# Probabilistic-Surgical-Vision/uncertainty-model

Hardware: AMD Instinct MI355X
Metric: stereo-pairs/sec (train step) at 256x512, 1/2/4/8 MI355X; loss delta vs ref (higher is better)
Workload: dtype bf16; 1 GPU; depth+uncertainty train step (BASELINE config 2): fwd+4-scale loss+bwd+Adam; global_batch=8, per_gpu_batch=8, height=256, width=512, loss=bayesian, parallelism=dp1, launch=hip-graph, graph=config.yml (nodes=5 stage graphs)

## Files before the change

### uncertainty-model_amd/csrc/knobs.h

```cpp
#pragma once

#define UM_KNOBS(X)                                                                         \
                                \
                \
  X(small, 1)                                                                               \
                \
                 \
                \
                  \
                           \
  X(small_tiles, 1024)                                                                      \
  X(split_below, 600)                                                                       \
  X(split_target, 1024)                                                                     \
  X(split_minsteps, 4)                                                                      \
                       \
                \
                     \
                  \
                   \
  X(glds_split_below, 256)                                                                  \
  X(glds_split_target, 512)                                                                 \
              \
  X(halo, 1)                                                                                \
  X(halo_min_tiles, 256)                                                                    \
                  \
                     \
  X(halo_max_nc, 192)                                                                       \
                       \
  X(odd_bn, 1)                                                                              \
              \
  X(bk64, 3)                                                                                \
                  \
                   \
                \
                    \
  X(glds, 5)                                                                                \
               \
                      \
                 \
                   \
  X(glds_deep, 3)                                                                           \
  X(glds_deep_blocks, 256)                                                                  \
                 \
                          \
  X(xcd_col, 0)                                                                             \
                 \
               \
             \
  X(tappack, 1)                                                                             \
                     \
  X(cls4, 1)                                                                                \
                  \
                 \
                    \
                \
              \
  X(cls_glds, 3)                                                                            \
                                            \
                   \
                 \
  X(pad_dgrad, 1)                                                                           \
                  \
                 \
                     \
                   \
                                                      \
  X(fold_split_nc, 64)                                                                      \
                                                   \
                             \
  X(halo_pf2, 0)                                                                            \
                    \
                 \
                    \
  X(halo_persist, 1)                                                                        \
  X(halo_grid, 0)                                                                           \
                  \
                   \
  X(halo_res_kb, 48)                                                                        \
                    \
  X(halo_staged, 1)                                                                         \
                    \
                      \
                                                         \
  X(border_valu, 1)                                                                         \
                       \
                        \
  X(s1x1, 1)                                                                                \
                   \
  X(s1x1_small, 1)                                                                          \
               \
                  \
  X(cat_fused, 0)                                                                           \
                   \
  X(merge_ns, 1)                                                                            \
              \
                                    \
  X(colred_single, 131072)                                                                  \
  X(colred_per, 16384)                                                                      \
               \
                                                          \
  X(wtr_tbk, 32)                                                                            \
                            \
  X(w1x1, 1)                                                                                \
               \
  X(border_split, 1)                                                                        \
                   \
  X(up2_valu, 1)                                                                            \
                   \
                                         \
  X(wsplit_blocks, 0)                                                                       \
                     \
  X(wred_t, 1)                                                                              \
                            \
  X(bn_bwd_rows_max, 1024)                                                                  \
                     \
  X(bn_slice, 1)                                                                            \
              \
                                          \
  X(dh_fwd, 0)                                                                              \
  X(dh_fwd128, 1)                                                                           \
               \
  X(dh_dgrad, 1)

namespace umamd {

struct Knobs {
#define UM_KNOB_FIELD(name, dflt) int name;
  UM_KNOBS(UM_KNOB_FIELD)
#undef UM_KNOB_FIELD
  Knobs();
};

Knobs& knobs();

}
```

### uncertainty-model_amd/csrc/wgrad_tr.hip

```cpp
#include <algorithm>
#include <cstdlib>

#include <atomic>

#include "common.h"
#include "wgrad_tr.h"
#include "knobs.h"

namespace {

typedef __attribute__((ext_vector_type(4))) __bf16 bf16x4_t;

constexpr int TBN = 128;

struct TrArgs {
  const bf16_t* x;
  const bf16_t* dy;
  float* slabs;
  int N, H, W, C, ldx, K, R, stride, pad, reflect, P, Q, ldy;
  int M, RRC, m_per_split;
  int row_step;
};

__device__ __forceinline__ int bit(int v, int b) { return (v >> b) & 1; }
template <int NCH>
__device__ __forceinline__ int swz(int row) {
  if (NCH == 8) return bit(row, 0) | (bit(row, 1) << 1) | (bit(row, 3) << 2);
  if (NCH == 4) return bit(row, 1) | (bit(row, 3) << 1);
  return 0;
}
template <int NCH>
__device__ __forceinline__ int img_off(int row, int c8) {
  return row * NCH * 16 + (((c8 >> 1) ^ swz<NCH>(row)) << 4) + ((c8 & 1) << 3);
}

__device__ __forceinline__ bf16x4_t tr_read(const bf16_t* p) {
  return __builtin_amdgcn_ds_read_tr16_b64_v4bf16(
      (__attribute__((address_space(3))) bf16x4_t*)(p));
}

struct Pix {
  int n, p, q;
  bool ok;
};
__device__ __forceinline__ Pix pix_at(long m, int P, int Q, long mend) {
  Pix x;
  x.ok = m < mend;
  const long mm = x.ok ? m : 0;
  const long pq = (long)P * Q;
  x.n = (int)(mm / pq);
  const int r = (int)(mm - x.n * pq);
  x.p = r / Q;
  x.q = r - x.p * Q;
  return x;
}
template <int BM, int TBK>
__global__ void __launch_bounds__(256) wgrad_tr_kernel(TrArgs a) {
  constexpr int NCA = BM / 16, NCB = TBN / 16;
  constexpr int TM = BM / 32, TN = 4;
  constexpr int A_PER = TBK * BM / 8 / 256;
  constexpr int B_PER = TBK * TBN / 8 / 256;
  constexpr int KS = TBK / 32;
  static_assert(A_PER >= 1 && B_PER >= 2 && TBK % 32 == 0, "tiles");
  __shared__ __attribute__((aligned(16))) bf16_t sA[2][TBK * BM];
  __shared__ __attribute__((aligned(16))) bf16_t sB[2][TBK * TBN];

  const int tid = threadIdx.x, lane = tid & 63, wave = tid >> 6;
  const int wm = wave >> 1, wn = wave & 1;
  const int g = lane >> 4, q4 = (lane >> 2) & 3, p4 = lane & 3;
  const int bk = blockIdx.x * BM;
  const int bj = blockIdx.y * TBN;
  const long m_begin = (long)blockIdx.z * a.m_per_split;
  const long m_end = min((long)a.M, m_begin + a.m_per_split);

  const int mlen = (int)(m_end - m_begin);
  int mrel = 0;
  const bf16_t* adp[A_PER];
  int aso[A_PER], alim[A_PER];
  const long astep = (long)TBK * a.ldy;
#pragma unroll
  for (int u = 0; u < A_PER; ++u) {
    const int id = tid + u * 256;
    const int row = id / (BM / 8), c8 = id % (BM / 8);
    aso[u] = img_off<NCA>(row, c8);
    alim[u] = bk + c8 * 8 < a.K ? mlen - row : 0;
    adp[u] = a.dy + (m_begin + row) * a.ldy + bk + c8 * 8;
  }
  const bf16_t* bimg[B_PER];
  int bso[B_PER], blim[B_PER], bp[B_PER], bq[B_PER], by0[B_PER], bx0[B_PER], byo[B_PER],
      bxo[B_PER];
  const long img_stride = (long)a.H * a.W * a.ldx;
  const int row_pitch = a.W * a.ldx;
  auto yoff = [&](int p, int y0) {
    int yy = p * a.stride + y0;
    if (a.reflect) yy = reflect_idx(yy, a.H);
    return (yy < 0 || yy >= a.H) ? -1 : yy * row_pitch;
  };
  auto xoff = [&](int q, int x0) {
    int xx = q * a.stride + x0;
    if (a.reflect) xx = reflect_idx(xx, a.W);
    return (xx < 0 || xx >= a.W) ? -1 : xx * a.ldx;
  };
#pragma unroll
  for (int u = 0; u < B_PER; ++u) {
    const int id = tid + u * 256;
    const int row = id / (TBN / 8), c8 = id % (TBN / 8);
    bso[u] = img_off<NCB>(row, c8);
    const int j = bj + c8 * 8;
    const bool ok = j < a.RRC;
    blim[u] = ok ? mlen - row : 0;
    const int jj = ok ? j : 0;
    const int tap = jj / a.C;
    const int ry = tap / a.R;
    by0[u] = ry - a.pad;
    bx0[u] = tap - ry * a.R - a.pad;
    const Pix px = pix_at(m_begin + row, a.P, a.Q, m_end);
    bp[u] = px.p;
    bq[u] = px.q;
    bimg[u] = a.x + px.n * img_stride + (jj - tap * a.C);
    byo[u] = yoff(bp[u], by0[u]);
    bxo[u] = xoff(bq[u], bx0[u]);
  }

  uint4 ra[A_PER], rb[B_PER];
  auto load = [&]() {
#pragma unroll
    for (int u = 0; u < A_PER; ++u) {
      ra[u] = make_uint4(0, 0, 0, 0);
      if (mrel < alim[u]) ra[u] = *reinterpret_cast<const uint4*>(adp[u]);
    }
#pragma unroll
    for (int u = 0; u < B_PER; ++u) {
      rb[u] = make_uint4(0, 0, 0, 0);
      if (mrel < blim[u] && (byo[u] | bxo[u]) >= 0)
        rb[u] = *reinterpret_cast<const uint4*>(bimg[u] + (byo[u] + bxo[u]));
    }
  };
  auto store = [&](int buf) {
#pragma unroll
    for (int u = 0; u < A_PER; ++u) *reinterpret_cast<uint4*>(&sA[buf][aso[u]]) = ra[u];
#pragma unroll
    for (int u = 0; u < B_PER; ++u) *reinterpret_cast<uint4*>(&sB[buf][bso[u]]) = rb[u];
  };
  auto advance = [&]() {
    mrel += TBK;
#pragma unroll
    for (int u = 0; u < A_PER; ++u) adp[u] += astep;
    const bool rows = a.row_step > 0;
#pragma unroll
    for (int u = 0; u < B_PER; ++u) {
      int p = bp[u], q = bq[u];
      const bf16_t* img = bimg[u];
      if (rows) {
        p += a.row_step;
        if (p >= a.P) {
          p -= a.P;
          img += img_stride;
        }
      } else {
        q += TBK;
        while (q >= a.Q) {
          q -= a.Q;
          if (++p == a.P) {
            p = 0;
            img += img_stride;
          }
        }
      }
      bp[u] = p;
      bq[u] = q;
      bimg[u] = img;
      byo[u] = yoff(p, by0[u]);
      if (!rows) bxo[u] = xoff(q, bx0[u]);
    }
  };

  int oa[TM][2], ob[TN][2];
#pragma unroll
  for (int h = 0; h < 2; ++h) {
    const int row = 8 * g + q4 + 4 * h;
#pragma unroll
    for (int i = 0; i < TM; ++i) {
      const int ct = (wm * (BM / 2) + i * 16) / 16;
      oa[i][h] = row * NCA * 16 + ((ct ^ swz<NCA>(row)) << 4) + 4 * p4;
    }
#pragma unroll
    for (int j = 0; j < TN; ++j) {
      const int ct = (wn * 64 + j * 16) / 16;
      ob[j][h] = row * NCB * 16 + ((ct ^ swz<NCB>(row)) << 4) + 4 * p4;
    }
  }

  f32x4_t acc[TM][TN];
#pragma unroll
  for (int i = 0; i < TM; ++i)
#pragma unroll
    for (int j = 0; j < TN; ++j) acc[i][j] = f32x4_t{0.f, 0.f, 0.f, 0.f};

  if (m_begin < m_end) {
    load();
    store(0);
    advance();
  }
  __syncthreads();
  int cur = 0;
  for (long m0 = m_begin; m0 < m_end; m0 += TBK) {
    const bool more = m0 + TBK < m_end;
    if (more) load();
#pragma unroll
    for (int ks = 0; ks < KS; ++ks) {
      const int da = ks * 32 * NCA * 16, db = ks * 32 * NCB * 16;
      bf16x8_t fa[TM], fb[TN];
#pragma unroll
      for (int i = 0; i < TM; ++i) {
        const bf16x4_t lo = tr_read(&sA[cur][oa[i][0] + da]);
        const bf16x4_t hi = tr_read(&sA[cur][oa[i][1] + da]);
        fa[i] = bf16x8_t{lo[0], lo[1], lo[2], lo[3], hi[0], hi[1], hi[2], hi[3]};
      }
#pragma unroll
      for (int j = 0; j < TN; ++j) {
        const bf16x4_t lo = tr_read(&sB[cur][ob[j][0] + db]);
        const bf16x4_t hi = tr_read(&sB[cur][ob[j][1] + db]);
        fb[j] = bf16x8_t{lo[0], lo[1], lo[2], lo[3], hi[0], hi[1], hi[2], hi[3]};
      }
#pragma unroll
      for (int i = 0; i < TM; ++i)
#pragma unroll
        for (int j = 0; j < TN; ++j)
          acc[i][j] = __builtin_amdgcn_mfma_f32_16x16x32_bf16(fa[i], fb[j], acc[i][j], 0, 0, 0);
    }
    if (more) {
      store(cur ^ 1);
      advance();
    }
    __syncthreads();
    cur ^= 1;
  }

  float* out = a.slabs + (long)blockIdx.z * a.K * a.RRC;
  const int col = lane & 15, row4 = (lane >> 4) * 4;
#pragma unroll
  for (int i = 0; i < TM; ++i)
#pragma unroll
    for (int j = 0; j < TN; ++j)
#pragma unroll
      for (int e = 0; e < 4; ++e) {
        const int k = bk + wm * (BM / 2) + i * 16 + row4 + e;
        const int jj = bj + wn * 64 + j * 16 + col;
        if (k < a.K && jj < a.RRC) out[(long)k * a.RRC + jj] = acc[i][j][e];
      }
}

}

namespace umamd {

int wgrad_tr_bm(int K) { return K <= 64 ? 64 : 128; }

int wgrad_tr_tbk() {
  const int t = knobs().wtr_tbk;
  return (t == 64 || t == 128) ? t : 32;
}

int wgrad_tr_blocks_per_cu(int K) {
  const int bm = wgrad_tr_bm(K), tbk = wgrad_tr_tbk();
  static std::atomic<int> cache[2][3] = {{{0}, {0}, {0}}, {{0}, {0}, {0}}};
  std::atomic<int>& slot = cache[bm == 128][tbk == 32 ? 0 : (tbk == 64 ? 1 : 2)];
  if (const int c = slot.load(std::memory_order_relaxed)) return c;
  const void* f = nullptr;
#define UM_WTRF(BM_, TBK_) \
  if (bm == BM_ && tbk == TBK_) f = reinterpret_cast<const void*>(&wgrad_tr_kernel<BM_, TBK_>);
  UM_WTRF(64, 32) UM_WTRF(64, 64) UM_WTRF(64, 128)
  UM_WTRF(128, 32) UM_WTRF(128, 64) UM_WTRF(128, 128)
#undef UM_WTRF
  int n = 0;
  if (f == nullptr || hipOccupancyMaxActiveBlocksPerMultiprocessor(&n, f, 256, 0) != hipSuccess) {
    (void)hipGetLastError();
    n = 1;
  }
  n = std::max(1, n);
  slot.store(n, std::memory_order_relaxed);
  return n;
}

int wgrad_tr_run(const void* x, int N, int H, int W, int C, int ldx, int K, int R, int stride,
                 int pad, int reflect, int P, int Q, const void* dy, int ldy, float* slabs,
                 int splits, hipStream_t st) {
  TrArgs a{};
  a.x = reinterpret_cast<const bf16_t*>(x);
  a.dy = reinterpret_cast<const bf16_t*>(dy);
  a.slabs = slabs;
  a.N = N; a.H = H; a.W = W; a.C = C; a.ldx = ldx; a.K = K; a.R = R; a.stride = stride;
  a.pad = pad; a.reflect = reflect; a.P = P; a.Q = Q; a.ldy = ldy;
  a.M = N * P * Q;
  a.RRC = R * R * C;
  if ((long)H * W * ldx > 0x7fffffffl) {
    umamd::set_error("wgrad_tr: an image of %d x %d x %d elements exceeds 32-bit offsets", H, W, ldx);
    return UM_ERR_ARG;
  }
  const int tbk = wgrad_tr_tbk();
  a.m_per_split = ceil_div(ceil_div(a.M, splits), tbk) * tbk;
  a.row_step = (tbk % Q == 0 && tbk / Q <= P) ? tbk / Q : 0;
  const int bm = wgrad_tr_bm(K);
  dim3 grid(ceil_div(K, bm), ceil_div(a.RRC, TBN), splits);
#define UM_WTR(BM_, TBK_)                                                                 \
  if (bm == BM_ && tbk == TBK_) {                                                         \
    hipLaunchKernelGGL((wgrad_tr_kernel<BM_, TBK_>), grid, dim3(256), 0, st, a);          \
    UM_LAUNCH_CHECK();                                                                    \
    return UM_OK;                                                                         \
  }
  UM_WTR(64, 32) UM_WTR(64, 64) UM_WTR(64, 128)
  UM_WTR(128, 32) UM_WTR(128, 64) UM_WTR(128, 128)
#undef UM_WTR
  umamd::set_error("wgrad_tr: no kernel for bm %d tbk %d", bm, tbk);
  return UM_ERR_ARG;
}

}
```

Before: 980.7 stereo-pairs/sec.

## Precompute im2col gather offsets in an LDS table for transposed wgrad

Replaces the per-thread pixel/tap coordinate tracking and bounds checks in the wgrad_tr B-operand loader with a shared-memory table of precomputed element offsets. The table covers a window of M rows and is rebuilt cooperatively when that window is exhausted. Out-of-bounds loads are redirected to a global zero page rather than being predicated. The aim is to cut integer/address arithmetic and branching in the inner load loop. The cost is extra LDS, periodic table rebuilds with a barrier, and a reworked 32-bit offset overflow check.

New measurement: 982.8 stereo-pairs/sec (median of 2 runs). Within noise of the previous version (+0.2%).

```diff
diff --git a/uncertainty-model_amd/csrc/knobs.h b/uncertainty-model_amd/csrc/knobs.h
--- a/uncertainty-model_amd/csrc/knobs.h
+++ b/uncertainty-model_amd/csrc/knobs.h
@@ -100,6 +100,9 @@
                \
                                                           \
   X(wtr_tbk, 32)                                                                            \
+                 \
+                                               \
+  X(wtr_win, 0)                                                                             \
                             \
   X(w1x1, 1)                                                                                \
                \
diff --git a/uncertainty-model_amd/csrc/wgrad_tr.hip b/uncertainty-model_amd/csrc/wgrad_tr.hip
--- a/uncertainty-model_amd/csrc/wgrad_tr.hip
+++ b/uncertainty-model_amd/csrc/wgrad_tr.hip
@@ -10,6 +10,7 @@
 namespace {
 
 typedef __attribute__((ext_vector_type(4))) __bf16 bf16x4_t;
+typedef __attribute__((ext_vector_type(4))) unsigned int u32x4_t;
 
 constexpr int TBN = 128;
 
@@ -19,7 +20,7 @@
   float* slabs;
   int N, H, W, C, ldx, K, R, stride, pad, reflect, P, Q, ldy;
   int M, RRC, m_per_split;
-  int row_step;
+  int win;
 };
 
 __device__ __forceinline__ int bit(int v, int b) { return (v >> b) & 1; }
@@ -39,21 +40,10 @@
       (__attribute__((address_space(3))) bf16x4_t*)(p));
 }
 
-struct Pix {
-  int n, p, q;
-  bool ok;
-};
-__device__ __forceinline__ Pix pix_at(long m, int P, int Q, long mend) {
-  Pix x;
-  x.ok = m < mend;
-  const long mm = x.ok ? m : 0;
-  const long pq = (long)P * Q;
-  x.n = (int)(mm / pq);
-  const int r = (int)(mm - x.n * pq);
-  x.p = r / Q;
-  x.q = r - x.p * Q;
-  return x;
-}
+__device__ __attribute__((aligned(16))) unsigned int g_wtr_zero[4];
+
+constexpr int tab_entries(int tbk) { return tbk == 128 ? 4096 : 2048; }
+
 template <int BM, int TBK>
 __global__ void __launch_bounds__(256) wgrad_tr_kernel(TrArgs a) {
   constexpr int NCA = BM / 16, NCB = TBN / 16;
@@ -64,6 +54,7 @@
   static_assert(A_PER >= 1 && B_PER >= 2 && TBK % 32 == 0, "tiles");
   __shared__ __attribute__((aligned(16))) bf16_t sA[2][TBK * BM];
   __shared__ __attribute__((aligned(16))) bf16_t sB[2][TBK * TBN];
+  __shared__ int stab[tab_entries(TBK)];
 
   const int tid = threadIdx.x, lane = tid & 63, wave = tid >> 6;
   const int wm = wave >> 1, wn = wave & 1;
@@ -75,104 +66,106 @@
 
   const int mlen = (int)(m_end - m_begin);
   int mrel = 0;
+  const bf16_t* const zero = reinterpret_cast<const bf16_t*>(g_wtr_zero);
   const bf16_t* adp[A_PER];
   int aso[A_PER], alim[A_PER];
-  const long astep = (long)TBK * a.ldy;
+  const bool a_ok = bk + (tid % (BM / 8)) * 8 < a.K;
+  const long astep = a_ok ? (long)TBK * a.ldy : 0;
 #pragma unroll
   for (int u = 0; u < A_PER; ++u) {
     const int id = tid + u * 256;
     const int row = id / (BM / 8), c8 = id % (BM / 8);
     aso[u] = img_off<NCA>(row, c8);
-    alim[u] = bk + c8 * 8 < a.K ? mlen - row : 0;
-    adp[u] = a.dy + (m_begin + row) * a.ldy + bk + c8 * 8;
-  }
-  const bf16_t* bimg[B_PER];
-  int bso[B_PER], blim[B_PER], bp[B_PER], bq[B_PER], by0[B_PER], bx0[B_PER], byo[B_PER],
-      bxo[B_PER];
-  const long img_stride = (long)a.H * a.W * a.ldx;
-  const int row_pitch = a.W * a.ldx;
-  auto yoff = [&](int p, int y0) {
-    int yy = p * a.stride + y0;
-    if (a.reflect) yy = reflect_idx(yy, a.H);
-    return (yy < 0 || yy >= a.H) ? -1 : yy * row_pitch;
-  };
-  auto xoff = [&](int q, int x0) {
-    int xx = q * a.stride + x0;
-    if (a.reflect) xx = reflect_idx(xx, a.W);
-    return (xx < 0 || xx >= a.W) ? -1 : xx * a.ldx;
-  };
+    alim[u] = mlen - row;
+    adp[u] = a_ok ? a.dy + (m_begin + row) * a.ldy + bk + c8 * 8 : zero;
+  }
+  const int pq = a.P * a.Q;
+  const int n0 = (int)(m_begin / pq);
+  const int tap0 = bj / a.C;
+  const int ntap = (min(bj + TBN, a.RRC) - 1) / a.C - tap0 + 1;
+  const int ld8 = a.ldx >> 3;
+  int wbase = 0;
+  auto build = [&]() {
+    const int wl = min(a.win, (mlen - wbase + TBK - 1) / TBK * TBK);
+    const int ry0 = tap0 / a.R, rx0 = tap0 - ry0 * a.R;
+    for (int w = tid; w < wl; w += 256) {
+      const long ml = m_begin + wbase + w;
+      const bool ok = ml < m_end;
+      const int m = (int)ml;
+      const int n = ok ? m / pq : 0;
+      const int r = ok ? m - n * pq : 0;
+      const int p = r / a.Q, q = r - p * a.Q;
+      const int ybase = p * a.stride - a.pad, xbase = q * a.stride - a.pad;
+      int ry = ry0, rx = rx0;
+      for (int t = 0; t < ntap; ++t) {
+        int yy = ybase + ry, xx = xbase + rx;
+        if (a.reflect) {
+          yy = reflect_idx(yy, a.H);
+          xx = reflect_idx(xx, a.W);
+        }
+        const bool in = ok && yy >= 0 && yy < a.H && xx >= 0 && xx < a.W;
+        stab[t * a.win + w] = in ? (((n - n0) * a.H + yy) * a.W + xx) * ld8 : -1;
+        if (++rx == a.R) {
+          rx = 0;
+          ++ry;
+        }
+      }
+    }
+  };
+  int bso[B_PER], tb[B_PER];
+  const int bc8 = tid % (TBN / 8);
+  const int bcol = bj + bc8 * 8;
+  const bool b_ok = bcol < a.RRC;
+  const int btap = b_ok ? bcol / a.C : tap0;
+  const char* const zpage = reinterpret_cast<const char*>(g_wtr_zero);
+  const char* const bbase =
+      b_ok ? reinterpret_cast<const char*>(a.x + (long)n0 * a.H * a.W * a.ldx + (bcol - btap * a.C))
+           : zpage;
+  const unsigned bmul = b_ok ? 16 : 0;
 #pragma unroll
   for (int u = 0; u < B_PER; ++u) {
-    const int id = tid + u * 256;
-    const int row = id / (TBN / 8), c8 = id % (TBN / 8);
-    bso[u] = img_off<NCB>(row, c8);
-    const int j = bj + c8 * 8;
-    const bool ok = j < a.RRC;
-    blim[u] = ok ? mlen - row : 0;
-    const int jj = ok ? j : 0;
-    const int tap = jj / a.C;
-    const int ry = tap / a.R;
-    by0[u] = ry - a.pad;
-    bx0[u] = tap - ry * a.R - a.pad;
-    const Pix px = pix_at(m_begin + row, a.P, a.Q, m_end);
-    bp[u] = px.p;
-    bq[u] = px.q;
-    bimg[u] = a.x + px.n * img_stride + (jj - tap * a.C);
-    byo[u] = yoff(bp[u], by0[u]);
-    bxo[u] = xoff(bq[u], bx0[u]);
-  }
-
-  uint4 ra[A_PER], rb[B_PER];
+    const int row = (tid + u * 256) / (TBN / 8);
+    bso[u] = img_off<NCB>(row, bc8);
+    tb[u] = (btap - tap0) * a.win + row;
+  }
+
+  u32x4_t ra[A_PER], rb[B_PER];
   auto load = [&]() {
-#pragma unroll
-    for (int u = 0; u < A_PER; ++u) {
-      ra[u] = make_uint4(0, 0, 0, 0);
-      if (mrel < alim[u]) ra[u] = *reinterpret_cast<const uint4*>(adp[u]);
-    }
+    if (mrel - wbase >= a.win) {
+      wbase = mrel;
+      build();
+      __syncthreads();
+    }
+    const int wrel = mrel - wbase;
+    int e[B_PER];
+#pragma unroll
+    for (int u = 0; u < B_PER; ++u) e[u] = stab[tb[u] + wrel];
+#pragma unroll
+    for (int u = 0; u < A_PER; ++u) ra[u] = *reinterpret_cast<const u32x4_t*>(adp[u]);
 #pragma unroll
     for (int u = 0; u < B_PER; ++u) {
-      rb[u] = make_uint4(0, 0, 0, 0);
-      if (mrel < blim[u] && (byo[u] | bxo[u]) >= 0)
-        rb[u] = *reinterpret_cast<const uint4*>(bimg[u] + (byo[u] + bxo[u]));
+      const char* src = bbase + (unsigned long)(unsigned)e[u] * bmul;
+      rb[u] = *reinterpret_cast<const u32x4_t*>(e[u] < 0 ? zpage : src);
+    }
+  };
+  auto clip = [&]() {
+    if (mrel + TBK > mlen) {
+#pragma unroll
+      for (int u = 0; u < A_PER; ++u)
+        if (mrel >= alim[u]) adp[u] = zero;
     }
   };
   auto store = [&](int buf) {
 #pragma unroll
-    for (int u = 0; u < A_PER; ++u) *reinterpret_cast<uint4*>(&sA[buf][aso[u]]) = ra[u];
-#pragma unroll
-    for (int u = 0; u < B_PER; ++u) *reinterpret_cast<uint4*>(&sB[buf][bso[u]]) = rb[u];
+    for (int u = 0; u < A_PER; ++u) *reinterpret_cast<u32x4_t*>(&sA[buf][aso[u]]) = ra[u];
+#pragma unroll
+    for (int u = 0; u < B_PER; ++u) *reinterpret_cast<u32x4_t*>(&sB[buf][bso[u]]) = rb[u];
   };
   auto advance = [&]() {
     mrel += TBK;
 #pragma unroll
     for (int u = 0; u < A_PER; ++u) adp[u] += astep;
-    const bool rows = a.row_step > 0;
-#pragma unroll
-    for (int u = 0; u < B_PER; ++u) {
-      int p = bp[u], q = bq[u];
-      const bf16_t* img = bimg[u];
-      if (rows) {
-        p += a.row_step;
-        if (p >= a.P) {
-          p -= a.P;
-          img += img_stride;
-        }
-      } else {
-        q += TBK;
-        while (q >= a.Q) {
-          q -= a.Q;
-          if (++p == a.P) {
-            p = 0;
-            img += img_stride;
-          }
-        }
-      }
-      bp[u] = p;
-      bq[u] = q;
-      bimg[u] = img;
-      byo[u] = yoff(p, by0[u]);
-      if (!rows) bxo[u] = xoff(q, bx0[u]);
-    }
+    clip();
   };
 
   int oa[TM][2], ob[TN][2];
@@ -198,14 +191,17 @@
     for (int j = 0; j < TN; ++j) acc[i][j] = f32x4_t{0.f, 0.f, 0.f, 0.f};
 
   if (m_begin < m_end) {
+    build();
+    clip();
+    __syncthreads();
     load();
     store(0);
     advance();
   }
   __syncthreads();
   int cur = 0;
-  for (long m0 = m_begin; m0 < m_end; m0 += TBK) {
-    const bool more = m0 + TBK < m_end;
+  for (int m0 = 0; m0 < mlen; m0 += TBK) {
+    const bool more = m0 + TBK < mlen;
     if (more) load();
 #pragma unroll
     for (int ks = 0; ks < KS; ++ks) {
@@ -294,13 +290,17 @@
   a.pad = pad; a.reflect = reflect; a.P = P; a.Q = Q; a.ldy = ldy;
   a.M = N * P * Q;
   a.RRC = R * R * C;
-  if ((long)H * W * ldx > 0x7fffffffl) {
-    umamd::set_error("wgrad_tr: an image of %d x %d x %d elements exceeds 32-bit offsets", H, W, ldx);
-    return UM_ERR_ARG;
-  }
   const int tbk = wgrad_tr_tbk();
   a.m_per_split = ceil_div(ceil_div(a.M, splits), tbk) * tbk;
-  a.row_step = (tbk % Q == 0 && tbk / Q <= P) ? tbk / Q : 0;
+  const long span = std::min<long>(N, ceil_div(a.m_per_split, P * Q) + 1);
+  if (span * H * W * (ldx / 8) > 0x7fffffffl) {
+    umamd::set_error("wgrad_tr: %ld images of %d x %d x %d elements exceed 32-bit offsets", span, H,
+                     W, ldx);
+    return UM_ERR_ARG;
+  }
+  const int taps = std::min(R * R, (TBN - 1) / C + 2);
+  a.win = tab_entries(tbk) / taps / tbk * tbk;
+  if (const int w = knobs().wtr_win; w > 0) a.win = std::min(a.win, ceil_div(w, tbk) * tbk);
   const int bm = wgrad_tr_bm(K);
   dim3 grid(ceil_div(K, bm), ceil_div(a.RRC, TBN), splits);
 #define UM_WTR(BM_, TBK_)                                                                 \
```
